# JiuTongBro/MultiView_Inpaint

Measured on AMD Instinct MI355X. Metric: Mpix/s fwd+bwd @1.5M Gauss 1080p, higher is better.
Workload: dtype f32; 1 GPU; rasterizer-with-depth fwd+bwd, one 1920x1080 view per GPU per step, N=1500000 Gaussians, sh_degree 3 (BASELINE.json configs[2] size, SURVEY.md §8d scene); gaussians=1500000, visible=1312313, num_rendered_D=14779663, tiles=8160, tile_list_max=2266, parallelism=views x1

## Files before the change

include/mvi_raster.h:

```cpp
#ifndef MVI_RASTER_H
#define MVI_RASTER_H

#include <stddef.h>
#include <stdint.h>

#ifdef __cplusplus
extern "C" {
#endif

#define MVI_OK 0
#define MVI_EINVAL (-1)
#define MVI_EHIP (-2)
#define MVI_ENOMEM (-3)

#define MVI_TILE 16

typedef struct mvi_raster_settings {
    int32_t image_height;
    int32_t image_width;
    float tanfovx;
    float tanfovy;
    float scale_modifier;
    int32_t sh_degree;
    int32_t prefiltered;
// ... 83 lines not shown
int mvi_raster_backward_geom_range(const mvi_raster_settings* s, int32_t P, int32_t M, int32_t first, int32_t count,
                                   const float* means3D, const float* shs, const float* colors_precomp, const float* scales,
                                   const float* rotations, const float* cov3D_precomp, const int32_t* radii, const void* geom,
                                   const float* grad_rows_scratch, float* dL_dmeans3D, float* dL_dmeans2D, float* dL_dopacity,
                                   float* dL_dshs, float* dL_dcolors, float* dL_dscales, float* dL_drotations, float* dL_dcov3D,
                                   void* stream);

typedef struct mvi_raster_views {
    const float* depths;
    const float* means2D;
    const float* cov3D_a;
    const float* cov3D_b;
    const float* conic_opacity;
    const float* rgbd;
    const uint32_t* tiles_touched;
    const uint8_t* clamped;
    const void* tile_ids_sorted;
    const uint32_t* point_list;
    const uint32_t* ranges;
    const float* final_T;
    const uint32_t* n_contrib;
    int32_t tile_id_bytes;
    const uint8_t* grad_support;
} mvi_raster_views;
int mvi_raster_get_views(int32_t P, int64_t num_rendered, int32_t image_width, int32_t image_height,
                         const void* geom, const void* binning, const void* image,
                         mvi_raster_views* out);
int mvi_raster_materialize_geom_views(const mvi_raster_settings* s, int32_t P, const float* means3D, const float* scales,
                                      const float* rotations, const float* cov3D_precomp, const int32_t* radii, void* geom,
                                      void* stream);
int mvi_raster_materialize_tile_ids(int32_t P, int64_t num_rendered, int32_t image_width, int32_t image_height,
                                    void* binning, const void* image, void* stream);

#define MVI_RASTER_NSTAGES 8
int mvi_raster_timing_enable(int enable);
int mvi_raster_timing_enable_stages(uint32_t stage_mask);
int mvi_raster_timing_read(float* ms_sum_host, int32_t* calls_host);
const char* mvi_raster_stage_name(int stage);

int mvi_raster_color_mode(int deferred);
int mvi_raster_forward_group(int group);
int mvi_raster_resolve_colors(const mvi_raster_settings* s, int32_t P, void* geom, size_t geom_bytes, void* stream);

int mvi_raster_binning_version(int version);
int mvi_raster_backward_mode(int dense);
int mvi_raster_dev_stamps(int pass, void* device_buffer);
int mvi_raster_dev_wave_sum9(const float* in, float* out, int n_waves, void* stream);

const char* mvi_raster_last_error(void);
const char* mvi_version(void);

#ifdef __cplusplus
}
#endif
#endif
```

multiview_inpaint_amd/_lib.py:

```python
import ctypes as C
import os
import re

_HERE = os.path.dirname(os.path.abspath(__file__))
LIB_PATH = os.environ.get("MVI_HIP_LIB") or os.path.join(_HERE, "csrc", "libmvi_hip.so")
LIB_OVERRIDDEN = bool(os.environ.get("MVI_HIP_LIB"))
if LIB_OVERRIDDEN:
    import sys as _sys
    _sys.stderr.write(f"[mvi] MVI_HIP_LIB is set: every kernel comes from {LIB_PATH}, not from the in-tree build\n")
INCLUDE_DIR = os.path.normpath(os.path.join(_HERE, "..", "include"))


class RasterSettings(C.Structure):
    _fields_ = [
        ("image_height", C.c_int32), ("image_width", C.c_int32),
        ("tanfovx", C.c_float), ("tanfovy", C.c_float), ("scale_modifier", C.c_float),
        ("sh_degree", C.c_int32), ("prefiltered", C.c_int32),
        ("bg", C.c_void_p), ("viewmatrix", C.c_void_p), ("projmatrix", C.c_void_p), ("campos", C.c_void_p),
    ]


class RasterViews(C.Structure):
    _fields_ = [(n, C.c_void_p) for n in (
        "depths", "means2D", "cov3D_a", "cov3D_b", "conic_opacity", "rgbd", "tiles_touched", "clamped",
        "tile_ids_sorted", "point_list", "ranges", "final_T", "n_contrib")] + [("tile_id_bytes", C.c_int32),
                                                                                   ("grad_support", C.c_void_p)]


class AdamGroup(C.Structure):
    _fields_ = [("param", C.c_void_p), ("grad", C.c_void_p), ("exp_avg", C.c_void_p), ("exp_avg_sq", C.c_void_p),
                ("n", C.c_int64), ("lr", C.c_float)]


class CompactTensor(C.Structure):
    _fields_ = [("in_", C.c_void_p), ("out", C.c_void_p), ("width", C.c_int32), ("packed_stride", C.c_int32)]


def declared_symbols():
    names = []
    for fn in sorted(os.listdir(INCLUDE_DIR)):
        if fn.endswith(".h"):
            src = open(os.path.join(INCLUDE_DIR, fn)).read()
            src = re.sub(r"/\*.*?\*/", "", src, flags=re.S)
            names += re.findall(r"\b(mvi_[a-z0-9_]+)\s*\(", src)
    return sorted(set(names))


def raster_source_digest():
    import hashlib
# ... 62 lines not shown
    L.mvi_raster_mark_visible.argtypes = [i32, vp, vp, vp, vp, vp]
    L.mvi_raster_get_views.restype = C.c_int
    L.mvi_raster_get_views.argtypes = [i32, i64, i32, i32, vp, vp, vp, C.POINTER(RasterViews)]
    L.mvi_raster_materialize_geom_views.restype = C.c_int
    L.mvi_raster_materialize_geom_views.argtypes = [C.POINTER(RasterSettings), i32] + [vp] * 7
    L.mvi_raster_materialize_tile_ids.restype = C.c_int
    L.mvi_raster_materialize_tile_ids.argtypes = [i32, i64, i32, i32, vp, vp, vp]
    L.mvi_raster_timing_enable.restype = C.c_int
    L.mvi_raster_timing_enable.argtypes = [C.c_int]
    L.mvi_raster_timing_enable_stages.restype = C.c_int
    L.mvi_raster_timing_enable_stages.argtypes = [C.c_uint32]
    L.mvi_raster_timing_read.restype = C.c_int
    L.mvi_raster_timing_read.argtypes = [C.POINTER(C.c_float), C.POINTER(C.c_int32)]
    L.mvi_raster_stage_name.restype = C.c_char_p
    L.mvi_raster_stage_name.argtypes = [C.c_int]
    L.mvi_raster_binning_version.restype = C.c_int
    L.mvi_raster_binning_version.argtypes = [C.c_int]
    L.mvi_raster_backward_mode.restype = C.c_int
    L.mvi_raster_backward_mode.argtypes = [C.c_int]
    L.mvi_raster_color_mode.restype = C.c_int
    L.mvi_raster_color_mode.argtypes = [C.c_int]
    L.mvi_raster_forward_group.restype = C.c_int
    L.mvi_raster_forward_group.argtypes = [C.c_int]
    L.mvi_raster_resolve_colors.restype = C.c_int
    L.mvi_raster_resolve_colors.argtypes = [C.POINTER(RasterSettings), i32, vp, sz, vp]
    L.mvi_raster_dev_stamps.restype = C.c_int
    L.mvi_raster_dev_stamps.argtypes = [C.c_int, vp]
    L.mvi_raster_dev_wave_sum9.restype = C.c_int
    L.mvi_raster_dev_wave_sum9.argtypes = [vp, vp, C.c_int, vp]
    _bind_unet_ops(L)
    _bind_train_ops(L)
    _bind_box_region(L)
    _lib = L
    return L


def _bind_unet_ops(L):
    try:
        from . import _unet_ops_bind
    except ImportError:
        return
    _unet_ops_bind.bind(L)


def _bind_train_ops(L):
    vp, i32, sz, f32 = C.c_void_p, C.c_int32, C.c_size_t, C.c_float
# ... 50 lines not shown
```

multiview_inpaint_amd/csrc/raster_api.hip:

```cpp
#include <cstdio>
#include <cstdlib>
#include <cstring>
#include <mutex>
#include <vector>

#include "raster_common.h"

static thread_local char g_err[512] = "";
static int g_dense_backward = [] { const char* e = getenv("MVI_RASTER_DENSE_BACKWARD"); return (e && e[0] == '1') ? 1 : 0; }();
static int g_defer_colors = [] { const char* e = getenv("MVI_RASTER_EAGER_COLORS"); return (e && e[0] == '1') ? 0 : 1; }();
namespace {
struct SegmentHint { const void* geom; int32_t P; int64_t segments; uint64_t stamp; };
constexpr int kSegmentHints = 64;
SegmentHint g_seg_hints[kSegmentHints] = {};
uint64_t g_seg_clock = 0;
std::mutex g_seg_mutex;
void remember_segments(const void* geom, int32_t P, int64_t segments) {
    std::lock_guard<std::mutex> lock(g_seg_mutex);
    int slot = 0;
    for (int i = 0; i < kSegmentHints; ++i) {
        if (g_seg_hints[i].geom == geom) { slot = i; break; }
        if (g_seg_hints[i].stamp < g_seg_hints[slot].stamp) slot = i;
    }
    g_seg_hints[slot] = {geom, P, segments, ++g_seg_clock};
// ... 81 lines not shown
    g_recs.clear();
    return MVI_OK;
}
const char* mvi_raster_stage_name(int i) {
    static const char* n[MVI_RASTER_NSTAGES] = {"preprocess_forward", "scan_block_sums", "duplicate_keys", "radix_sort",
                                                "tile_ranges", "render_forward", "render_backward", "preprocess_backward"};
    return (i >= 0 && i < MVI_RASTER_NSTAGES) ? n[i] : "";
}
int mvi_raster_dev_stamps(int pass, void* device_buffer) { mvi::set_dev_stamps(pass, device_buffer); return MVI_OK; }
int mvi_raster_dev_wave_sum9(const float* in, float* out, int n_waves, void* stream) {
    if (n_waves < 0 || (n_waves > 0 && (!in || !out))) return fail(MVI_EINVAL, "wave_sum9: NULL buffer or negative n_waves%s");
    if (mvi::launch_wave_sum9_probe(in, out, n_waves, (hipStream_t)stream)) return hip_fail("wave_sum9 probe", hipGetLastError());
    return MVI_OK;
}
int mvi_raster_backward_mode(int dense) {
    const int old = g_dense_backward;
    if (dense == 0 || dense == 1) g_dense_backward = dense;
    return old;
}
int mvi_raster_binning_version(int version) { return mvi::set_binning_version(version); }
int mvi_raster_forward_group(int group) {
    const int old = mvi::set_forward_group(group);
    return old < 0 ? fail(MVI_EINVAL, "forward group: no such instantiation of render_forward%s") : old;
}
int mvi_raster_color_mode(int deferred) {
    const int old = g_defer_colors;
    if (deferred == 0 || deferred == 1) g_defer_colors = deferred;
    return old;
}
int mvi_raster_resolve_colors(const mvi_raster_settings* s, int32_t P, void* geom, size_t geom_bytes, void* stream) {
    mvi::Frame f;
    if (int rc = make_frame(s, P, 0, f)) return rc;
    if (P == 0) return MVI_OK;
    if (!geom) return fail(MVI_EINVAL, "geom is NULL%s");
    mvi::GeomView g = mvi::carve_geom(geom, P);
    if (geom_bytes < g.bytes) return fail(MVI_ENOMEM, "geom scratch too small%s", "");
    if (mvi::launch_resolve_colors(f, g, (hipStream_t)stream)) return hip_fail("resolve_colors", hipGetLastError());
    return MVI_OK;
}
const char* mvi_version(void) { return "multiview_inpaint_amd 0.1.0 (gfx950)"; }

size_t mvi_raster_geom_bytes(int32_t P) { return mvi::carve_geom(nullptr, P).bytes; }
size_t mvi_raster_image_bytes(int32_t W, int32_t H) { return mvi::carve_image(nullptr, W, H).bytes; }
size_t mvi_raster_binning_bytes(int64_t D, int32_t W, int32_t H) { return mvi::carve_binning(nullptr, D, W, H).bytes; }

static int forward_geom_impl(const mvi_raster_settings* s, mvi::Frame& f, int32_t P, int32_t M, const float* means3D,
// ... 410 lines not shown
}

int mvi_raster_get_views(int32_t P, int64_t D, int32_t W, int32_t H, const void* geom, const void* binning,
                         const void* image, mvi_raster_views* out) {
    if (!out) return fail(MVI_EINVAL, "views is NULL%s");
    memset(out, 0, sizeof(*out));
    if (geom) {
        mvi::GeomView g = mvi::carve_geom(const_cast<void*>(geom), P);
        out->depths = g.depths; out->means2D = reinterpret_cast<const float*>(g.xy);
        out->cov3D_a = reinterpret_cast<const float*>(g.cov_a); out->cov3D_b = reinterpret_cast<const float*>(g.cov_b);
        out->conic_opacity = reinterpret_cast<const float*>(g.conic_opacity); out->rgbd = reinterpret_cast<const float*>(g.rgbd);
        out->tiles_touched = g.tiles_touched; out->clamped = g.clamped;
        out->grad_support = g.touched;
    }
    if (binning) {
        mvi::BinningView b = mvi::carve_binning(const_cast<void*>(binning), D, W, H);
        int fin = b.passes & 1;
        out->tile_ids_sorted = b.keys[fin]; out->point_list = b.vals[fin];
        out->tile_id_bytes = b.key_bytes;
    }
    if (image) {
        mvi::ImageView im = mvi::carve_image(const_cast<void*>(image), W, H);
        out->ranges = im.ranges; out->final_T = im.final_T; out->n_contrib = im.n_contrib;
    }
    return MVI_OK;
}

int mvi_raster_materialize_geom_views(const mvi_raster_settings* s, int32_t P, const float* means3D, const float* scales,
                                      const float* rotations, const float* cov3D_precomp, const int32_t* radii, void* geom,
                                      void* stream) {
    mvi::Frame f;
    if (int rc = make_frame(s, P, 0, f)) return rc;
    if (P == 0) return MVI_OK;
    if (!means3D || !radii || !geom) return fail(MVI_EINVAL, "NULL means3D/radii/geom in materialize_geom_views%s");
    if (((scales == nullptr) || (rotations == nullptr)) == (cov3D_precomp == nullptr))
        return fail(MVI_EINVAL, "Please provide exactly one of either scale/rotation pair or precomputed 3D covariance!%s");
    mvi::GeomView g = mvi::carve_geom(geom, P);
    if (mvi::launch_materialize_geom_views(f, means3D, scales, rotations, cov3D_precomp, radii, g, (hipStream_t)stream))
        return hip_fail("materialize_geom_views", hipGetLastError());
    return MVI_OK;
}

int mvi_raster_materialize_tile_ids(int32_t P, int64_t D, int32_t W, int32_t H, void* binning, const void* image, void* stream) {
    if (P < 0 || D < 0 || W < 0 || H < 0) return fail(MVI_EINVAL, "negative size in materialize_tile_ids%s");
    if (P == 0 || D == 0) return MVI_OK;
    if (!binning || !image) return fail(MVI_EINVAL, "NULL scratch in materialize_tile_ids%s");
// ... 9 lines not shown
```

multiview_inpaint_amd/csrc/raster_binning.hip:

```cpp
#include "raster_common.h"
#include "raster_scan.h"

namespace mvi {

__global__ __launch_bounds__(256) void zero_fill_kernel(uint4* __restrict__ p, size_t n16) {
    for (size_t i = (size_t)blockIdx.x * 256 + threadIdx.x; i < n16; i += (size_t)gridDim.x * 256) p[i] = make_uint4(0u, 0u, 0u, 0u);
}
int launch_zero_fill(void* p, size_t bytes, hipStream_t st) {
    if (bytes == 0) return 0;
    const size_t n16 = (bytes + 15) / 16;
    size_t blocks = (n16 + 255) / 256;
    if (blocks > 256 * 32) blocks = 256 * 32;
    hipLaunchKernelGGL(zero_fill_kernel, dim3((unsigned)blocks), dim3(256), 0, st, (uint4*)p, n16);
    return hipGetLastError() == hipSuccess ? 0 : MVI_EHIP;
}

__global__ __launch_bounds__(1024) void scan_block_sums_kernel(const uint32_t* __restrict__ sums,
                                                               uint32_t* __restrict__ offsets, int n) {
    __shared__ uint32_t s_wave[16];
    __shared__ uint32_t s_carry;
    const int tid = threadIdx.x;
    const uint32_t total = row_excl_scan_1024(sums, offsets, n, tid, s_wave, &s_carry);
    if (tid == 0) offsets[n] = total;
}
// ... 325 lines not shown
    {
        StageTimer tm(kStDup, st);
        hipLaunchKernelGGL((emit_pairs_kernel<KeyT>), dim3(nblk), dim3(kBlock), 0, st, f, g, g.dvals[0], g.perm_offsets,
                           keys[0], b.vals[0]);
    }
    int cur = 0;
    {
        StageTimer tm(kStSort, st);
        int shift = 0;
        for (int p = 0; p < b.passes; ++p) {
            const int left = b.passes - p;
            const int bits = (b.key_bits - shift + left - 1) / left;
            cur = radix_pass<kSortWavesD, KeyT>(keys, b.vals, cur, D, shift, bits, b.block_hist, b.digit_tot, b.nsort, st);
            shift += bits;
        }
    }
    int nrb = (int)((D + kBlock - 1) / kBlock);
    StageTimer tm(kStRanges, st);
    hipLaunchKernelGGL((tile_ranges_kernel<KeyT>), dim3(nrb), dim3(kBlock), 0, st, keys[cur], D, im.ranges);
    return hipGetLastError() == hipSuccess ? 0 : MVI_EHIP;
}

int launch_binning(const Frame& f, GeomView g, BinningView b, ImageView im, int64_t D, hipStream_t st) {
    size_t tiles = (size_t)f.gx * f.gy;
    if (launch_zero_fill(im.ranges, 8 * tiles, st)) return MVI_EHIP;
    if (D <= 0 || f.P <= 0) return 0;
    return b.key_bytes == 2 ? binning_typed<uint16_t>(f, g, b, im, D, st) : binning_typed<uint32_t>(f, g, b, im, D, st);
}

}
```

multiview_inpaint_amd/csrc/raster_binning2.hip:

```cpp
#include <cstdlib>

#include "raster_common.h"
#include "raster_scan.h"

namespace mvi {

static int g_binning_version = [] { const char* e = getenv("MVI_BINNING_LEGACY"); return (e && e[0] == '1') ? 1 : 2; }();
bool binning_v2_enabled() { return g_binning_version == 2; }
int set_binning_version(int v) {
    const int old = g_binning_version;
    if (v == 1 || v == 2) g_binning_version = v;
    return old;
}

__device__ __forceinline__ uint32_t block_excl_scan256(uint32_t v, int tid, uint32_t* s_w4, uint32_t* total) {
    const int lane = tid & 63, wave = tid >> 6;
    const uint32_t inc = wave_incl_scan(v, lane);
    if (wave < 4 && lane == 63) s_w4[wave] = inc;
    __syncthreads();
    uint32_t off = 0;
#pragma unroll
    for (int w = 0; w < 3; ++w) if (w < wave) off += s_w4[w];
    if (total) *total = s_w4[0] + s_w4[1] + s_w4[2] + s_w4[3];
    __syncthreads();
// ... 314 lines not shown
    if (!load_chunk(chunk_first, col_start, gx, tid, s_first, s_col, ck)) return;
    const uint32_t last = ck.seg1 ? ck.seg1 - 1u : 0u;
    uint32_t yhs[kEx2Items];
#pragma unroll
    for (int k = 0; k < kEx2Items; ++k) yhs[k] = seg_yh[min(ck.seg0 + (uint32_t)(k * kExThreads + tid), last)];
#pragma unroll
    for (int k = 0; k < kEx2Items; ++k) {
        const uint32_t i = ck.seg0 + (uint32_t)(k * kExThreads + tid);
        if (i < ck.seg1) {
            const uint32_t yh = yhs[k];
            const uint32_t y0 = yh & 255u, h = (yh >> 8) + 1u;
            atomicAdd(&s_d[y0], 1u);
            atomicSub(&s_d[y0 + h], 1u);
        }
    }
    __syncthreads();
    const uint32_t v = tid < 256 ? s_d[tid] : 0u;
    const uint32_t ex = block_excl_scan256(v, tid, s_w4, nullptr);
    if (tid < gy) row_table[(size_t)tid * stride + blockIdx.x] = ex + v;
}

__global__ __launch_bounds__(1024) void row_scan_kernel(int gx, const uint32_t* __restrict__ chunk_first,
                                                        uint32_t* __restrict__ row_table, int stride,
                                                        uint32_t* __restrict__ row_tot, uint32_t* __restrict__ col_rel) {
    __shared__ uint32_t s_first[257];
    __shared__ uint32_t s_wave[16];
    __shared__ uint32_t s_carry;
    const int tid = threadIdx.x;
    if (tid <= gx) s_first[tid] = chunk_first[tid];
    const int n = (int)chunk_first[gx];
    uint32_t* row = row_table + (size_t)blockIdx.x * stride;
    const uint32_t total = row_excl_scan_1024(row, row, n, tid, s_wave, &s_carry);
    __syncthreads();
    uint32_t* cr = col_rel + (size_t)blockIdx.x * (gx + 1);
    if (tid < gx) cr[tid] = __hip_atomic_load(row + s_first[tid], __ATOMIC_RELAXED, __HIP_MEMORY_SCOPE_AGENT);
    if (tid == 0) { cr[gx] = total; row_tot[blockIdx.x] = total; }
}

struct ExpandArgs {
    int n_items;
    int nbins;
    int gx;
    const uint32_t* order;
    const uint2* rect_sorted;
    const uint32_t* chunk_first;
    const uint32_t* col_start;
    const uint32_t* seg_idx_in;
    const uint16_t* seg_yh_in;
    const uint32_t* col_rel;
    uint32_t* ranges;
    const uint32_t* table;
// ... 188 lines not shown

int launch_binning2_level1(const Frame& f, GeomView g, hipStream_t st) {
    if (f.P <= 0) return 0;
    {
        StageTimer tm(kStSort, st);
#define MVI_DS_PASS(PASS, SRC, DST)                                                                                              \
        hipLaunchKernelGGL(depth_count_kernel, dim3(g.nds), dim3(kDsThreads), 0, st, g.dkeys[SRC], f.P, 8 * PASS, g.ds_table,     \
                           g.ds_super[PASS & 1]);                                                                                 \
        hipLaunchKernelGGL((depth_scatter_kernel<PASS>), dim3(g.nds), dim3(kDsThreads), 0, st, g.dkeys[SRC], g.dvals[SRC],        \
                           g.dkeys[DST], g.dvals[DST], f.P, g.ds_table, g.ds_super[PASS & 1], g.nsuper,                           \
                           PASS < 3 ? g.ds_super[(PASS + 1) & 1] : (uint32_t*)nullptr, g.rect, g.rect_sorted);
        MVI_DS_PASS(0, 0, 1) MVI_DS_PASS(1, 1, 0) MVI_DS_PASS(2, 0, 1) MVI_DS_PASS(3, 1, 0)
#undef MVI_DS_PASS
    }
    StageTimer tm(kStDup, st);
    hipLaunchKernelGGL(column_count_kernel, dim3(g.nblk1), dim3(kExThreads), 0, st, f.P, f.gx, g.rect_sorted, g.col_table,
                       g.nblk1);
    hipLaunchKernelGGL(columns_scan_kernel, dim3(f.gx), dim3(1024), 0, st, g.col_table, g.nblk1, g.nblk1, g.col_tot, f.gx,
                       g.arrivals, g.chunk_first, g.col_start);
    return hipGetLastError() == hipSuccess ? 0 : MVI_EHIP;
}

int launch_binning2(const Frame& f, GeomView g, BinningView b, ImageView im, int64_t D, int64_t segments, hipStream_t st) {
    const size_t tiles = (size_t)f.gx * f.gy;
    if (D <= 0 || f.P <= 0) return launch_zero_fill(im.ranges, 8 * tiles, st);
    const bool wide = f.gx > 128 || f.gy > 128;
    ExpandArgs a1{};
    a1.n_items = f.P; a1.nbins = f.gx; a1.gx = f.gx;
    a1.order = g.dvals[0]; a1.rect_sorted = g.rect_sorted;
    a1.table = g.col_table; a1.tot = g.col_tot; a1.stride = g.nblk1;
    a1.out_idx = b.vals[0]; a1.out_aux = (uint16_t*)b.keys[0];
    a1.stamps = g_dev_stamps[0];
    {
        StageTimer tm(kStDup, st);
        if (wide)
            hipLaunchKernelGGL((expand_scatter_kernel<1, 256, kExItems, 64 * 256>), dim3(g.nblk1), dim3(kExThreads), 0, st, a1);
        else hipLaunchKernelGGL((expand_scatter_kernel<1, 128, kExItems, 64 * 128>), dim3(g.nblk1), dim3(kExThreads), 0, st, a1);
    }
    int nchunk = b.nsort;
    if (segments > 0 && segments <= D) nchunk = (int)min((int64_t)b.nsort, segments / kEx2Chunk + f.gx + 1);
    ExpandArgs a2{};
    a2.nbins = f.gy; a2.gx = f.gx;
    a2.chunk_first = g.chunk_first; a2.col_start = g.col_start;
    a2.seg_idx_in = b.vals[0]; a2.seg_yh_in = (const uint16_t*)b.keys[0];
    a2.col_rel = b.col_rel; a2.ranges = im.ranges;
    a2.table = b.block_hist; a2.tot = b.digit_tot; a2.stride = b.nsort;
    a2.out_idx = b.vals[1];
    a2.stamps = g_dev_stamps[1];
    StageTimer tm(kStSort, st);
    hipLaunchKernelGGL(row_count_kernel, dim3(nchunk), dim3(kExThreads), 0, st, f.gx, f.gy, g.chunk_first, g.col_start,
                       (const uint16_t*)b.keys[0], b.block_hist, b.nsort);
    hipLaunchKernelGGL(row_scan_kernel, dim3(f.gy), dim3(1024), 0, st, f.gx, g.chunk_first, b.block_hist, b.nsort,
                       b.digit_tot, b.col_rel);
    if (f.gy <= kEx2SmallNB)
        hipLaunchKernelGGL((expand_scatter_kernel<2, kEx2SmallNB, kEx2Items, kEx2SmallCap>), dim3(nchunk), dim3(kExThreads), 0,
                           st, a2);
    else if (f.gy <= 128)
        hipLaunchKernelGGL((expand_scatter_kernel<2, 128, kEx2Items, 64 * 128>), dim3(nchunk), dim3(kExThreads), 0, st, a2);
    else hipLaunchKernelGGL((expand_scatter_kernel<2, 256, kEx2Items, 64 * 256>), dim3(nchunk), dim3(kExThreads), 0, st, a2);
    return hipGetLastError() == hipSuccess ? 0 : MVI_EHIP;
}

}
```

multiview_inpaint_amd/csrc/raster_common.h:

```cpp
#pragma once
#include <hip/hip_runtime.h>
#include <stdint.h>
#include <stddef.h>
#include <type_traits>

#include "../../include/mvi_raster.h"

namespace mvi {

constexpr int kTile = MVI_TILE;
constexpr int kBlock = 256;
constexpr int kPB = 64;
constexpr float kNearZ = 0.2f;
constexpr float kLowpass = 0.3f;
constexpr float kFrustumClamp = 1.3f;
constexpr float kLambdaFloor = 0.1f;
constexpr float kAlphaMax = 0.99f;
constexpr float kAlphaMin = 1.0f / 255.0f;
constexpr float kTEps = 0.0001f;
constexpr float kDepthSentinel = 15.0f;

constexpr int kSortItems = 8;
constexpr int kSortWavesP = 4;
constexpr int kSortWavesD = 8;
// ... 12 lines not shown
    const float* campos;
    const float* bg;
    const float* shs_rest = nullptr;
    int raw = 0;
    int bin_v2 = 0;
    int defer_colors = 0;
};

constexpr int kDsThreads = 256;
constexpr int kDsItems = 8;
constexpr int kDsTile = kDsThreads * kDsItems;
constexpr int kDsSuper = 16;
constexpr int kExThreads = 512;
constexpr int kExItems = 4;
constexpr int kExChunk = kExThreads * kExItems;
constexpr int kEx2Items = 3;
constexpr int kEx2Chunk = kExThreads * kEx2Items;
constexpr int kEx2SmallNB = 80;
constexpr int kEx2SmallCap = 7168;
bool binning_v2_enabled();
void set_dev_stamps(int pass, void* buf);
int set_binning_version(int v);
int set_forward_group(int g);
inline bool binning_v2_ok(int gx, int gy) { return gx <= 256 && gy <= 256 && binning_v2_enabled(); }

struct ColorSource {
    const float* means3D;
    const float* shs;
    const float* shs_rest;
    int32_t M, deg, raw;
    int32_t deferred;
    int32_t vec16;
};

struct GeomView {
    float* depths;
    float2* xy;
    float4* cov_a;
    float2* cov_b;
    float4* conic_opacity;
    float4* rgbd;
    uint32_t* tiles_touched;
    uint2* rect;
    uint8_t* clamped;
    uint8_t* front;
    struct ColorSource* color_src;
    uint8_t* touched;
    uint32_t* block_sums;
    uint32_t* block_offsets;
    uint32_t* dkeys[2];
    uint32_t* dvals[2];
    uint32_t* dhist;
    uint32_t* dtot;
    uint32_t* perm_sums;
    uint32_t* perm_offsets;
    uint2* rect_sorted;
    uint32_t* col_table;
    uint32_t* col_tot;
    uint32_t* seg_sums;
    uint32_t* chunk_first;
    uint32_t* col_start;
    uint32_t* arrivals;
    uint32_t* ds_table;
    uint32_t* ds_super[2];
    int nds, nsuper;
    int nblk1;
    int nsortP;
    size_t bytes;
};
struct ImageView {
    uint32_t* ranges;
    float* final_T;
    uint32_t* n_contrib;
    size_t bytes;
};
struct BinningView {
    void* keys[2];
    int key_bytes;
    uint32_t* vals[2];
    uint32_t* block_hist;
    uint32_t* digit_tot;
    int nsort;
    int passes;
    int key_bits;
    int v2;
    uint32_t* col_rel;
    size_t bytes;
};

inline size_t align256(size_t x) { return (x + 255) & ~size_t(255); }

inline GeomView carve_geom(void* base, int P) {
    GeomView g;
    char* p = (char*)base;
// ... 27 lines not shown
    g.nblk1 = (int)((n + kExChunk - 1) / kExChunk);
    g.col_table = (uint32_t*)take(4 * 256 * (size_t)g.nblk1);
    g.col_tot = (uint32_t*)take(4 * 256);
    g.seg_sums = (uint32_t*)take(4 * npre);
    g.chunk_first = (uint32_t*)take(4 * 257);
    g.col_start = (uint32_t*)take(4 * 257);
    g.arrivals = (uint32_t*)take(4);
    g.nds = (int)((n + kDsTile - 1) / kDsTile);
    g.nsuper = (g.nds + kDsSuper - 1) / kDsSuper;
    g.ds_table = (uint32_t*)take(4 * 256 * (size_t)g.nds);
    g.ds_super[0] = (uint32_t*)take(4 * 256 * (size_t)g.nsuper);
    g.ds_super[1] = (uint32_t*)take(4 * 256 * (size_t)g.nsuper);
    g.bytes = o;
    return g;
}
inline ImageView carve_image(void* base, int W, int H) {
    ImageView v;
    char* p = (char*)base;
    size_t o = 0;
    size_t tiles = (size_t)((W + kTile - 1) / kTile) * ((H + kTile - 1) / kTile);
    size_t px = (size_t)W * H;
    auto take = [&](size_t b) { char* r = p ? p + o : nullptr; o += align256(b); return r; };
    v.ranges = (uint32_t*)take(8 * (tiles ? tiles : 1));
    v.final_T = (float*)take(4 * (px ? px : 1));
    v.n_contrib = (uint32_t*)take(4 * (px ? px : 1));
    v.bytes = o;
    return v;
}
inline int tile_bits(int W, int H) {
    unsigned tiles = (unsigned)(((W + kTile - 1) / kTile) * ((H + kTile - 1) / kTile));
    int b = 0;
    while ((1u << b) < tiles && b < 31) ++b;
    return b > 0 ? b : 1;
}
inline BinningView carve_binning(void* base, int64_t D, int W, int H) {
    BinningView v;
    char* p = (char*)base;
    size_t o = 0;
    size_t n = (size_t)(D > 0 ? D : 1);
    v.nsort = sort_blocks(n, kSortWavesD);
    v.key_bits = tile_bits(W, H);
    v.passes = (v.key_bits + 7) / 8;
    auto take = [&](size_t b) { char* r = p ? p + o : nullptr; o += align256(b); return r; };
    const unsigned tiles = (unsigned)(((W + kTile - 1) / kTile) * ((H + kTile - 1) / kTile));
    v.key_bytes = tiles <= 65536u ? 2 : 4;
    const int gx = (W + kTile - 1) / kTile, gy = (H + kTile - 1) / kTile;
    v.v2 = binning_v2_ok(gx, gy) ? 1 : 0;
    v.col_rel = nullptr;
    if (v.v2) {
        v.nsort = (int)((n / kEx2Chunk + (size_t)gx + 1 + 3) / 4 * 4);
// ... 196 lines not shown
}
__device__ __forceinline__ bool color_pending(float4 cd) { return cd.x < 0.0f || cd.y < 0.0f || cd.z < 0.0f; }

template <int CTRL, int ROW_MASK>
__device__ __forceinline__ float dpp_add(float v) {
    int t = __builtin_amdgcn_update_dpp(0, __float_as_int(v), CTRL, ROW_MASK, 0xf, true);
    return v + __int_as_float(t);
}
__device__ __forceinline__ float wave_sum_to_lane63(float v) {
    v = dpp_add<0xb1, 0xf>(v);
    v = dpp_add<0x4e, 0xf>(v);
    v = dpp_add<0x114, 0xf>(v);
    v = dpp_add<0x118, 0xf>(v);
    v = dpp_add<0x142, 0xa>(v);
    v = dpp_add<0x143, 0xc>(v);
    return v;
}
__device__ __forceinline__ float row_sum_to_lane15(float v) {
    v = dpp_add<0xb1, 0xf>(v);
    v = dpp_add<0x4e, 0xf>(v);
    v = dpp_add<0x114, 0xf>(v);
    v = dpp_add<0x118, 0xf>(v);
    return v;
}
__device__ __forceinline__ uint32_t wave_sum_u32(uint32_t v) {
    for (int o = 32; o > 0; o >>= 1) v += __shfl_xor(v, o);
    return v;
}

enum Stage { kStPreFwd = 0, kStScan, kStDup, kStSort, kStRanges, kStRenderFwd, kStRenderBwd, kStPreBwd };
void stage_begin(int stage, hipStream_t st);
void stage_end(int stage, hipStream_t st);
struct StageTimer {
    int stage; hipStream_t st;
    StageTimer(int s, hipStream_t q) : stage(s), st(q) { stage_begin(stage, st); }
    ~StageTimer() { stage_end(stage, st); }
};

constexpr int kMaxZero = 10;
struct ZeroRegions {
    float* head[kMaxZero];
    uint4* body[kMaxZero];
    float* tail[kMaxZero];
    uint32_t n_head[kMaxZero], n_body[kMaxZero], n_tail[kMaxZero];
    int n = 0;
    bool overflow = false;
// ... 74 lines not shown
```

multiview_inpaint_amd/csrc/raster_render.hip:

```cpp
#include <cstdlib>

#include "raster_common.h"
#include "raster_render_shared.h"

namespace mvi {


template <int G, bool AUX>
__global__ __launch_bounds__(kBlock) __attribute__((amdgpu_waves_per_eu(G == 1 ? 1 : 6, G == 1 ? 8 : 6))) void render_forward_kernel(
    Frame f, const uint32_t* __restrict__ ranges, const uint32_t* __restrict__ point_list,
    const float2* __restrict__ xy, float4* rgbd, const float4* __restrict__ conic_opacity,
    float* __restrict__ final_T, uint32_t* __restrict__ n_contrib, float* __restrict__ out_color,
    float* __restrict__ out_depth, ZeroRegions zero, const ColorSource* __restrict__ color_src, uint8_t* clamped,
    float* __restrict__ out_expected_depth, float* __restrict__ out_alpha) {
    __shared__ float2 s_xy[kBlock];
    __shared__ float s_t2[kBlock];
    __shared__ float4 s_co[kBlock];
    __shared__ float4 s_cd[kBlock];
    __shared__ float4 w_s[4][3][64];
    const int tid = threadIdx.x, wave = tid >> 6, lane = tid & 63;
    zero_share(zero, tid, kBlock);
    const int tile = xcd_band_tile(blockIdx.x, f.gx * f.gy);
    const int tile_y = tile / f.gx, tile_x = tile - tile_y * f.gx;
    const int qx0 = tile_x * kTile + 8 * (wave & 1), qy0 = tile_y * kTile + 8 * (wave >> 1);
    const int pxi = qx0 + (lane & 7), pyi = qy0 + (lane >> 3);
    const bool inside = pxi < f.W && pyi < f.H;
    const float pfx = (float)pxi, pfy = (float)pyi;
    const uint32_t r0 = ranges[2 * tile], r1 = ranges[2 * tile + 1];
    int todo = (int)(r1 - r0);
    const int rounds = (todo + kBlock - 1) / kBlock;

    float T = inside ? 1.0f : 0.0f;
    float T_out = 1.0f, C2 = 0.f, Dp = kDepthSentinel, Tc = 1.0f;
    [[maybe_unused]] float Dexp = 0.f;
    f2 C01 = {0.f, 0.f};
    uint32_t last = 0;

// ... 66 lines not shown
            } else {
                const float4* g = &w_s[wave][0][0];
                int k = 0;
                float chain = 0.0f;
                if (cnt >= G) {
                    do {
                        float4 a = g[0], co = g[64], cd = g[128];
#pragma unroll
                        for (int j = 0; j < G; ++j) {
                            const int jn = j + 1 < G ? j + 1 : j;
                            const float4 an = g[jn], con = g[64 + jn], cdn = g[128 + jn];
                            __builtin_amdgcn_sched_barrier(0);
                            chain = entry(a, co, cd, chain);
                            a = an; co = con; cd = cdn;
                        }
                        k += G; g += G;
                    } while ((k + G <= cnt) & (ballot64(T > 0.0f) != 0ull));
                }
                if (k < cnt && ballot64(T > 0.0f) != 0ull)
                    for (; k < cnt; ++k, ++g) chain = entry(g[0], g[64], g[128], chain);
            }
        }
    }
    if (inside) {
        size_t pix = (size_t)pyi * f.W + pxi, hw = (size_t)f.H * f.W;
        final_T[pix] = T_out;
        n_contrib[pix] = last;
        out_color[pix] = C01.x + T_out * f.bg[0];
        out_color[hw + pix] = C01.y + T_out * f.bg[1];
        out_color[2 * hw + pix] = C2 + T_out * f.bg[2];
        out_depth[pix] = Tc < 0.5f ? Dp : kDepthSentinel;
        if constexpr (AUX) {
            out_expected_depth[pix] = Dexp;
            out_alpha[pix] = 1.0f - T_out;
        }
    }
}

constexpr int kFrontTiles = 4;
constexpr int kFrontMax = 1024;
__global__ __launch_bounds__(kBlock) void mark_front_kernel(int tiles, const uint32_t* __restrict__ ranges,
                                                            const uint32_t* __restrict__ point_list, uint8_t* __restrict__ front,
                                                            int n_front, const ColorSource* __restrict__ color_src, int gx,
                                                            int every) {
    if (!color_src->deferred) return;
    const int tid = threadIdx.x;
    const int sx = (gx + every - 1) / every;
#pragma unroll
    for (int t = 0; t < kFrontTiles; ++t) {
        const int j = blockIdx.x * kFrontTiles + t;
        const int tile = every == 1 ? j : (j / sx) * every * gx + (j % sx) * every;
        if (tile >= tiles) break;
        const uint32_t r0 = ranges[2 * tile], r1 = ranges[2 * tile + 1];
        const uint32_t n = min(r1 - r0, (uint32_t)n_front);
        for (uint32_t e = tid; e < n; e += kBlock) front[point_list[r0 + e]] = 1;
    }
}
constexpr int kMarkedPer = 4;
// ... 13 lines not shown
            if (((w >> (8 * k)) & 0xFFu) && i0 + k < f.P) s_id[atomicAdd(&s_n, 1u)] = (uint32_t)(i0 + k);
    }
    __syncthreads();
    const uint32_t total = s_n;
    for (uint32_t i = tid; i < total; i += kBlock) {
        const uint32_t id = s_id[i];
        const float4 cd = g.rgbd[id];
        if (color_pending(cd)) resolve_color(cs, f.campos, id, cd.w, g.rgbd, g.clamped);
    }
}

constexpr int kForwardGroupDefault = 4;
static bool forward_group_built(int g) { return g == 1 || g == 4; }
static int g_forward_group = [] { const char* e = getenv("MVI_RASTER_FORWARD_GROUP"); const int v = e ? atoi(e) : 0;
                                  return forward_group_built(v) ? v : kForwardGroupDefault; }();
int set_forward_group(int g) {
    const int old = g_forward_group;
    if (g == -1) return old;
    if (g != 0 && !forward_group_built(g)) return MVI_EINVAL;
    g_forward_group = g == 0 ? kForwardGroupDefault : g;
    return old;
}

int launch_zero_fill(void* p, size_t bytes, hipStream_t st);
int launch_render_forward(const Frame& f, GeomView g, BinningView b, ImageView im, int64_t D,
                          float* out_color, float* out_depth, hipStream_t st, float* zero_rows, float* out_expected_depth,
                          float* out_alpha) {
    if ((out_expected_depth == nullptr) != (out_alpha == nullptr)) return MVI_EINVAL;
    ZeroRegions z;
    if (zero_rows) {
        z.add(zero_rows, (size_t)f.P * kGradRow);
        z.add(g.touched, ((size_t)f.P + 15) / 16 * 4);
    }
    if (f.W <= 0 || f.H <= 0) return launch_zero_regions(z, st);
    const uint32_t* plist = b.vals[b.passes & 1];
    const unsigned blocks = (unsigned)(f.gx * f.gy);
    if (f.defer_colors && D > 0) {
        static const int n_front = [] { const char* e = getenv("MVI_RASTER_FRONT_ENTRIES"); const int v = e ? atoi(e) : kBlock;
                                        return v < 0 ? 0 : (v > kFrontMax ? kFrontMax : v); }();
        static const int every = [] { const char* e = getenv("MVI_RASTER_FRONT_EVERY"); const int v = e ? atoi(e) : 2; return v < 1 ? 1 : v; }();
        if (n_front > 0) {
            const unsigned sampled = (unsigned)(((f.gx + every - 1) / every) * ((f.gy + every - 1) / every));
            hipLaunchKernelGGL(mark_front_kernel, dim3((sampled + kFrontTiles - 1) / kFrontTiles), dim3(kBlock), 0, st, (int)blocks,
                               im.ranges, plist, g.front, n_front, g.color_src, f.gx, every);
            hipLaunchKernelGGL(resolve_marked_kernel, dim3((f.P + kBlock * kMarkedPer - 1) / (kBlock * kMarkedPer)), dim3(kBlock), 0, st,
                               f, g);
        }
    }
#define MVI_RENDER_FORWARD(G, AUX)                                                                                          \
    hipLaunchKernelGGL((render_forward_kernel<G, AUX>), dim3(blocks), dim3(kBlock), 0, st, f, im.ranges, plist, g.xy, g.rgbd, \
                       g.conic_opacity, im.final_T, im.n_contrib, out_color, out_depth, z, g.color_src, g.clamped,            \
                       out_expected_depth, out_alpha)
    switch (g_forward_group * 2 + (out_alpha ? 1 : 0)) {
        case 2: MVI_RENDER_FORWARD(1, false); break;
        case 3: MVI_RENDER_FORWARD(1, true); break;
        case 8: MVI_RENDER_FORWARD(4, false); break;
        case 9: MVI_RENDER_FORWARD(4, true); break;
        default: return MVI_EINVAL;
    }
#undef MVI_RENDER_FORWARD
    return hipGetLastError() == hipSuccess ? 0 : MVI_EHIP;
}

__global__ __launch_bounds__(256) void zero_regions_kernel(ZeroRegions z) { zero_share(z, threadIdx.x, 256); }
int launch_zero_regions(const ZeroRegions& z, hipStream_t st) {
    if (z.n == 0) return 0;
    hipLaunchKernelGGL(zero_regions_kernel, dim3(2048), dim3(256), 0, st, z);
    return hipGetLastError() == hipSuccess ? 0 : MVI_EHIP;
}


__global__ __launch_bounds__(64) void wave_sum9_probe_kernel(const float* __restrict__ in, float* __restrict__ out) {
    const int lane = threadIdx.x;
    const float* x = in + (size_t)blockIdx.x * 9 * 64 + lane;
    const float s = wave_sum9(x[0], x[64], x[128], x[192], x[256], x[320], x[384], x[448], x[512]);
    if (wave_sum9_owner(lane)) out[blockIdx.x * 9 + wave_sum9_moment(lane)] = s;
}
int launch_wave_sum9_probe(const float* in, float* out, int n_waves, hipStream_t st) {
    if (n_waves <= 0) return 0;
    hipLaunchKernelGGL(wave_sum9_probe_kernel, dim3(n_waves), dim3(64), 0, st, in, out);
    return hipGetLastError() == hipSuccess ? 0 : MVI_EHIP;
}

#ifndef MVI_RB_WAVES
#define MVI_RB_WAVES 5
#endif
__global__ __launch_bounds__(kB2) __attribute__((amdgpu_waves_per_eu(MVI_RB_WAVES, MVI_RB_WAVES))) void render_backward_kernel(
    Frame f, const uint32_t* __restrict__ ranges, const uint32_t* __restrict__ point_list,
    const float2* __restrict__ xy, const float4* __restrict__ rgbd, const float4* __restrict__ conic_opacity,
    const float* __restrict__ final_T, const uint32_t* __restrict__ n_contrib,
    const float* __restrict__ dL_dpix, float* __restrict__ grad_rows, uint8_t* __restrict__ touched, ZeroRegions zero) {
#pragma clang fp contract(off)
    zero_share(zero, threadIdx.x, kB2);
    __shared__ float4 s_ent[3][kB2];
    __shared__ float s_acc[kB2][9];
    __shared__ uint32_t s_blast[2];
    const int tid = threadIdx.x, wave = tid >> 6, lane = tid & 63;
    const int tile = xcd_band_tile(blockIdx.x, f.gx * f.gy);
    const int tile_y = tile / f.gx, tile_x = tile - tile_y * f.gx;
    const int hx0 = tile_x * kTile, hy0 = tile_y * kTile + 8 * wave;
    const int pxi = hx0 + (lane & 15), py0 = hy0 + 2 * (lane >> 4), py1 = py0 + 1;
    const bool in0 = pxi < f.W && py0 < f.H, in1 = pxi < f.W && py1 < f.H;
    const float pfx = (float)pxi;
    const f2 pfy = {(float)py0, (float)py1};
    const uint32_t r0 = ranges[2 * tile];
    const size_t hw = (size_t)f.H * f.W, pix0 = (size_t)py0 * f.W + pxi, pix1 = pix0 + f.W;

    const f2 T_final = {in0 ? final_T[pix0] : 0.0f, in1 ? final_T[pix1] : 0.0f};
    f2 T = T_final;
    const uint32_t last0 = in0 ? n_contrib[pix0] : 0u, last1 = in1 ? n_contrib[pix1] : 0u;
    f2 A_dot = {0.f, 0.f};
    f2 dp0 = {0.f, 0.f}, dp1 = {0.f, 0.f}, dp2 = {0.f, 0.f};
    if (in0) { dp0.x = dL_dpix[pix0]; dp1.x = dL_dpix[hw + pix0]; dp2.x = dL_dpix[2 * hw + pix0]; }
    if (in1) { dp0.y = dL_dpix[pix1]; dp1.y = dL_dpix[hw + pix1]; dp2.y = dL_dpix[2 * hw + pix1]; }
    const f2 bg_dot = f.bg[0] * dp0 + f.bg[1] * dp1 + f.bg[2] * dp2;
    const f2 bg_term = -T_final * bg_dot;
    uint32_t wave_last = max(last0, last1);
    for (int o = 32; o > 0; o >>= 1) wave_last = max(wave_last, (uint32_t)__shfl_xor((int)wave_last, o));
    if (lane == 0) s_blast[wave] = wave_last;
    __syncthreads();
    const int total = (int)max(s_blast[0], s_blast[1]);
// ... 95 lines not shown
                }
            }
            asm volatile("s_waitcnt lgkmcnt(0)" ::: "memory");
            __builtin_amdgcn_wave_barrier();
            const int comp = lane & 15;
#pragma unroll 4
            for (int it = 0; it < 16; ++it) {
                const int e = wave * 64 + it * 4 + (lane >> 4);
                const uint32_t id = e < n ? __float_as_uint(s_ent[0][e].w) : 0xFFFFFFFFu;
                if (id == 0xFFFFFFFFu || comp >= 9) continue;
                atomicAdd(&grad_rows[(size_t)id * kRow + comp], s_acc[e][comp]);
                if (comp == 0) touched[id] = 1;
            }
        }
    }
}

int launch_render_backward(const Frame& f, GeomView g, BinningView b, ImageView im, int64_t D,
                           const float* dL_dpix, float* grad_rows, hipStream_t st, const ZeroRegions* zero) {
    ZeroRegions z;
    if (zero) z = *zero;
    if (f.W <= 0 || f.H <= 0 || D <= 0) return launch_zero_regions(z, st);
    const uint32_t* plist = b.vals[b.passes & 1];
    hipLaunchKernelGGL(render_backward_kernel, dim3(f.gx * f.gy), dim3(kB2), 0, st, f, im.ranges, plist, g.xy,
                       g.rgbd, g.conic_opacity, im.final_T, im.n_contrib, dL_dpix, grad_rows, g.touched, z);
    return hipGetLastError() == hipSuccess ? 0 : MVI_EHIP;
}

}
```

Baseline: 2498 Mpix/s.

## Schedule backward render tiles heaviest-first via per-band tile-class queues

The forward kernel now takes the maximum contributor count of each tile and buckets the tile into one of 16 cost classes per XCD band, appending its id to a per-class queue through an atomic. The backward kernel maps block ids through these queues so the most expensive tiles launch first within each band, which is meant to reduce the tail imbalance at the end of the backward pass. In exchange it adds a wave max reduction, a syncthreads and an atomic to the forward pass, a slightly larger zero fill, and an extra lookup per backward block. The new order is on by default, with an env/API switch back to plain band order.

Result: faster. 2586 Mpix/s, median of 6 (+3.5%).

```diff
diff --git a/include/mvi_raster.h b/include/mvi_raster.h
--- a/include/mvi_raster.h
+++ b/include/mvi_raster.h
@@ -129,6 +129,8 @@
     const uint32_t* n_contrib;
     int32_t tile_id_bytes;
     const uint8_t* grad_support;
+    const uint32_t* tile_class_count;
+    const uint32_t* tile_class_queue;
 } mvi_raster_views;
 int mvi_raster_get_views(int32_t P, int64_t num_rendered, int32_t image_width, int32_t image_height,
                          const void* geom, const void* binning, const void* image,
@@ -147,6 +149,7 @@
 
 int mvi_raster_color_mode(int deferred);
 int mvi_raster_forward_group(int group);
+int mvi_raster_backward_order(int order);
 int mvi_raster_resolve_colors(const mvi_raster_settings* s, int32_t P, void* geom, size_t geom_bytes, void* stream);
 
 int mvi_raster_binning_version(int version);
diff --git a/multiview_inpaint_amd/_lib.py b/multiview_inpaint_amd/_lib.py
--- a/multiview_inpaint_amd/_lib.py
+++ b/multiview_inpaint_amd/_lib.py
@@ -24,7 +24,9 @@
     _fields_ = [(n, C.c_void_p) for n in (
         "depths", "means2D", "cov3D_a", "cov3D_b", "conic_opacity", "rgbd", "tiles_touched", "clamped",
         "tile_ids_sorted", "point_list", "ranges", "final_T", "n_contrib")] + [("tile_id_bytes", C.c_int32),
-                                                                                   ("grad_support", C.c_void_p)]
+                                                                                   ("grad_support", C.c_void_p),
+                                                                                   ("tile_class_count", C.c_void_p),
+                                                                                   ("tile_class_queue", C.c_void_p)]
 
 
 class AdamGroup(C.Structure):
@@ -133,6 +135,8 @@
     L.mvi_raster_color_mode.argtypes = [C.c_int]
     L.mvi_raster_forward_group.restype = C.c_int
     L.mvi_raster_forward_group.argtypes = [C.c_int]
+    L.mvi_raster_backward_order.restype = C.c_int
+    L.mvi_raster_backward_order.argtypes = [C.c_int]
     L.mvi_raster_resolve_colors.restype = C.c_int
     L.mvi_raster_resolve_colors.argtypes = [C.POINTER(RasterSettings), i32, vp, sz, vp]
     L.mvi_raster_dev_stamps.restype = C.c_int
diff --git a/multiview_inpaint_amd/csrc/raster_api.hip b/multiview_inpaint_amd/csrc/raster_api.hip
--- a/multiview_inpaint_amd/csrc/raster_api.hip
+++ b/multiview_inpaint_amd/csrc/raster_api.hip
@@ -127,6 +127,10 @@
 int mvi_raster_forward_group(int group) {
     const int old = mvi::set_forward_group(group);
     return old < 0 ? fail(MVI_EINVAL, "forward group: no such instantiation of render_forward%s") : old;
+}
+int mvi_raster_backward_order(int order) {
+    const int old = mvi::set_backward_order(order);
+    return old < 0 ? fail(MVI_EINVAL, "backward order: 1 (heaviest first), 0 (plain band order) or -1 (query)%s") : old;
 }
 int mvi_raster_color_mode(int deferred) {
     const int old = g_defer_colors;
@@ -583,6 +587,7 @@
     if (image) {
         mvi::ImageView im = mvi::carve_image(const_cast<void*>(image), W, H);
         out->ranges = im.ranges; out->final_T = im.final_T; out->n_contrib = im.n_contrib;
+        out->tile_class_count = im.class_count; out->tile_class_queue = im.class_queue;
     }
     return MVI_OK;
 }
diff --git a/multiview_inpaint_amd/csrc/raster_binning.hip b/multiview_inpaint_amd/csrc/raster_binning.hip
--- a/multiview_inpaint_amd/csrc/raster_binning.hip
+++ b/multiview_inpaint_amd/csrc/raster_binning.hip
@@ -371,8 +371,7 @@
 }
 
 int launch_binning(const Frame& f, GeomView g, BinningView b, ImageView im, int64_t D, hipStream_t st) {
-    size_t tiles = (size_t)f.gx * f.gy;
-    if (launch_zero_fill(im.ranges, 8 * tiles, st)) return MVI_EHIP;
+    if (launch_zero_fill(im.ranges, ranges_and_counts_bytes(im), st)) return MVI_EHIP;
     if (D <= 0 || f.P <= 0) return 0;
     return b.key_bytes == 2 ? binning_typed<uint16_t>(f, g, b, im, D, st) : binning_typed<uint32_t>(f, g, b, im, D, st);
 }
diff --git a/multiview_inpaint_amd/csrc/raster_binning2.hip b/multiview_inpaint_amd/csrc/raster_binning2.hip
--- a/multiview_inpaint_amd/csrc/raster_binning2.hip
+++ b/multiview_inpaint_amd/csrc/raster_binning2.hip
@@ -360,11 +360,13 @@
 
 __global__ __launch_bounds__(1024) void row_scan_kernel(int gx, const uint32_t* __restrict__ chunk_first,
                                                         uint32_t* __restrict__ row_table, int stride,
-                                                        uint32_t* __restrict__ row_tot, uint32_t* __restrict__ col_rel) {
+                                                        uint32_t* __restrict__ row_tot, uint32_t* __restrict__ col_rel,
+                                                        uint32_t* __restrict__ class_count) {
     __shared__ uint32_t s_first[257];
     __shared__ uint32_t s_wave[16];
     __shared__ uint32_t s_carry;
     const int tid = threadIdx.x;
+    if (blockIdx.x == 0 && tid < kTileBands * kTileClasses) class_count[tid] = 0u;
     if (tid <= gx) s_first[tid] = chunk_first[tid];
     const int n = (int)chunk_first[gx];
     uint32_t* row = row_table + (size_t)blockIdx.x * stride;
@@ -599,8 +601,7 @@
 }
 
 int launch_binning2(const Frame& f, GeomView g, BinningView b, ImageView im, int64_t D, int64_t segments, hipStream_t st) {
-    const size_t tiles = (size_t)f.gx * f.gy;
-    if (D <= 0 || f.P <= 0) return launch_zero_fill(im.ranges, 8 * tiles, st);
+    if (D <= 0 || f.P <= 0) return launch_zero_fill(im.ranges, ranges_and_counts_bytes(im), st);
     const bool wide = f.gx > 128 || f.gy > 128;
     ExpandArgs a1{};
     a1.n_items = f.P; a1.nbins = f.gx; a1.gx = f.gx;
@@ -628,7 +629,7 @@
     hipLaunchKernelGGL(row_count_kernel, dim3(nchunk), dim3(kExThreads), 0, st, f.gx, f.gy, g.chunk_first, g.col_start,
                        (const uint16_t*)b.keys[0], b.block_hist, b.nsort);
     hipLaunchKernelGGL(row_scan_kernel, dim3(f.gy), dim3(1024), 0, st, f.gx, g.chunk_first, b.block_hist, b.nsort,
-                       b.digit_tot, b.col_rel);
+                       b.digit_tot, b.col_rel, im.class_count);
     if (f.gy <= kEx2SmallNB)
         hipLaunchKernelGGL((expand_scatter_kernel<2, kEx2SmallNB, kEx2Items, kEx2SmallCap>), dim3(nchunk), dim3(kExThreads), 0,
                            st, a2);
diff --git a/multiview_inpaint_amd/csrc/raster_common.h b/multiview_inpaint_amd/csrc/raster_common.h
--- a/multiview_inpaint_amd/csrc/raster_common.h
+++ b/multiview_inpaint_amd/csrc/raster_common.h
@@ -58,6 +58,7 @@
 void set_dev_stamps(int pass, void* buf);
 int set_binning_version(int v);
 int set_forward_group(int g);
+int set_backward_order(int order);
 inline bool binning_v2_ok(int gx, int gy) { return gx <= 256 && gy <= 256 && binning_v2_enabled(); }
 
 struct ColorSource {
@@ -104,8 +105,15 @@
     int nsortP;
     size_t bytes;
 };
+constexpr int kTileBands = 8;
+constexpr int kTileClasses = 16;
+constexpr int kTileClassWidth = 32;
+__host__ __device__ inline int tile_queue_stride(int tiles) { return (tiles + kTileBands - 1) / kTileBands + 1; }
+template <typename T> __host__ __device__ inline T* tile_class_queues(T* class_count) { return class_count + kTileBands * kTileClasses; }
 struct ImageView {
     uint32_t* ranges;
+    uint32_t* class_count;
+    uint32_t* class_queue;
     float* final_T;
     uint32_t* n_contrib;
     size_t bytes;
@@ -179,10 +187,15 @@
     size_t px = (size_t)W * H;
     auto take = [&](size_t b) { char* r = p ? p + o : nullptr; o += align256(b); return r; };
     v.ranges = (uint32_t*)take(8 * (tiles ? tiles : 1));
+    v.class_count = (uint32_t*)take(4 * kTileBands * kTileClasses);
+    v.class_queue = (uint32_t*)take(4 * (size_t)kTileBands * kTileClasses * (size_t)tile_queue_stride((int)tiles));
     v.final_T = (float*)take(4 * (px ? px : 1));
     v.n_contrib = (uint32_t*)take(4 * (px ? px : 1));
     v.bytes = o;
     return v;
+}
+inline size_t ranges_and_counts_bytes(const ImageView& v) {
+    return (size_t)((char*)v.class_count - (char*)v.ranges) + 4 * (size_t)kTileBands * kTileClasses;
 }
 inline int tile_bits(int W, int H) {
     unsigned tiles = (unsigned)(((W + kTile - 1) / kTile) * ((H + kTile - 1) / kTile));
@@ -425,6 +438,19 @@
     v = dpp_add<0x114, 0xf>(v);
     v = dpp_add<0x118, 0xf>(v);
     return v;
+}
+template <int CTRL>
+__device__ __forceinline__ uint32_t dpp_umax(uint32_t v) {
+    return max(v, (uint32_t)__builtin_amdgcn_update_dpp(0, (int)v, CTRL, 0xf, 0xf, true));
+}
+__device__ __forceinline__ uint32_t wave_umax(uint32_t v) {
+    v = dpp_umax<0xb1>(v);
+    v = dpp_umax<0x4e>(v);
+    v = dpp_umax<0x114>(v);
+    v = dpp_umax<0x118>(v);
+    const uint32_t a = (uint32_t)__builtin_amdgcn_readlane((int)v, 15), b = (uint32_t)__builtin_amdgcn_readlane((int)v, 31);
+    const uint32_t c = (uint32_t)__builtin_amdgcn_readlane((int)v, 47), d = (uint32_t)__builtin_amdgcn_readlane((int)v, 63);
+    return max(max(a, b), max(c, d));
 }
 __device__ __forceinline__ uint32_t wave_sum_u32(uint32_t v) {
     for (int o = 32; o > 0; o >>= 1) v += __shfl_xor(v, o);
diff --git a/multiview_inpaint_amd/csrc/raster_render.hip b/multiview_inpaint_amd/csrc/raster_render.hip
--- a/multiview_inpaint_amd/csrc/raster_render.hip
+++ b/multiview_inpaint_amd/csrc/raster_render.hip
@@ -1,4 +1,5 @@
 #include <cstdlib>
+#include <mutex>
 
 #include "raster_common.h"
 #include "raster_render_shared.h"
@@ -12,7 +13,8 @@
     const float2* __restrict__ xy, float4* rgbd, const float4* __restrict__ conic_opacity,
     float* __restrict__ final_T, uint32_t* __restrict__ n_contrib, float* __restrict__ out_color,
     float* __restrict__ out_depth, ZeroRegions zero, const ColorSource* __restrict__ color_src, uint8_t* clamped,
-    float* __restrict__ out_expected_depth, float* __restrict__ out_alpha) {
+    float* __restrict__ out_expected_depth, float* __restrict__ out_alpha, uint32_t* __restrict__ class_count) {
+    __shared__ uint32_t s_wmax[4];
     __shared__ float2 s_xy[kBlock];
     __shared__ float s_t2[kBlock];
     __shared__ float4 s_co[kBlock];
@@ -125,6 +127,15 @@
             }
         }
     }
+    const uint32_t wmax = wave_umax(last);
+    if (lane == 0) s_wmax[wave] = wmax;
+    __syncthreads();
+    uint32_t cls = 0, slot = 0;
+    if (tid == 0) {
+        const uint32_t m = max(max(s_wmax[0], s_wmax[1]), max(s_wmax[2], s_wmax[3]));
+        cls = (blockIdx.x & (kTileBands - 1)) * kTileClasses + min((uint32_t)(kTileClasses - 1), m / kTileClassWidth);
+        slot = atomicAdd(&class_count[cls], 1u);
+    }
     if (inside) {
         size_t pix = (size_t)pyi * f.W + pxi, hw = (size_t)f.H * f.W;
         final_T[pix] = T_out;
@@ -137,6 +148,10 @@
             out_expected_depth[pix] = Dexp;
             out_alpha[pix] = 1.0f - T_out;
         }
+    }
+    if (tid == 0) {
+        const uint32_t stride = (uint32_t)tile_queue_stride(f.gx * f.gy);
+        if (slot < stride) tile_class_queues(class_count)[(size_t)cls * stride + slot] = (uint32_t)tile;
     }
 }
 
@@ -196,6 +211,39 @@
     return old;
 }
 
+constexpr int kBackwardOrderDefault = 1;
+static int g_backward_order = [] { const char* e = getenv("MVI_RASTER_BACKWARD_ORDER");
+                                   return e && (e[0] == '0' || e[0] == '1') && e[1] == 0 ? e[0] - '0' : kBackwardOrderDefault; }();
+int set_backward_order(int order) {
+    const int old = g_backward_order;
+    if (order == -1) return old;
+    if (order != 0 && order != 1) return MVI_EINVAL;
+    g_backward_order = order;
+    return old;
+}
+namespace {
+struct QueueNote { const void* image; int W, H; uint64_t stamp; };
+constexpr int kQueueNotes = 64;
+QueueNote g_queue_notes[kQueueNotes] = {};
+uint64_t g_queue_clock = 0;
+std::mutex g_queue_mutex;
+void note_queue_filled(const void* image, int W, int H) {
+    std::lock_guard<std::mutex> lock(g_queue_mutex);
+    int slot = 0;
+    for (int i = 0; i < kQueueNotes; ++i) {
+        if (g_queue_notes[i].image == image) { slot = i; break; }
+        if (g_queue_notes[i].stamp < g_queue_notes[slot].stamp) slot = i;
+    }
+    g_queue_notes[slot] = {image, W, H, ++g_queue_clock};
+}
+bool queue_filled(const void* image, int W, int H) {
+    std::lock_guard<std::mutex> lock(g_queue_mutex);
+    for (int i = 0; i < kQueueNotes; ++i)
+        if (g_queue_notes[i].image == image && g_queue_notes[i].stamp) return g_queue_notes[i].W == W && g_queue_notes[i].H == H;
+    return false;
+}
+}
+
 int launch_zero_fill(void* p, size_t bytes, hipStream_t st);
 int launch_render_forward(const Frame& f, GeomView g, BinningView b, ImageView im, int64_t D,
                           float* out_color, float* out_depth, hipStream_t st, float* zero_rows, float* out_expected_depth,
@@ -224,7 +272,7 @@
 #define MVI_RENDER_FORWARD(G, AUX)                                                                                          \
     hipLaunchKernelGGL((render_forward_kernel<G, AUX>), dim3(blocks), dim3(kBlock), 0, st, f, im.ranges, plist, g.xy, g.rgbd, \
                        g.conic_opacity, im.final_T, im.n_contrib, out_color, out_depth, z, g.color_src, g.clamped,            \
-                       out_expected_depth, out_alpha)
+                       out_expected_depth, out_alpha, im.class_count)
     switch (g_forward_group * 2 + (out_alpha ? 1 : 0)) {
         case 2: MVI_RENDER_FORWARD(1, false); break;
         case 3: MVI_RENDER_FORWARD(1, true); break;
@@ -233,7 +281,9 @@
         default: return MVI_EINVAL;
     }
 #undef MVI_RENDER_FORWARD
-    return hipGetLastError() == hipSuccess ? 0 : MVI_EHIP;
+    if (hipGetLastError() != hipSuccess) return MVI_EHIP;
+    note_queue_filled(im.ranges, f.W, f.H);
+    return 0;
 }
 
 __global__ __launch_bounds__(256) void zero_regions_kernel(ZeroRegions z) { zero_share(z, threadIdx.x, 256); }
@@ -259,18 +309,36 @@
 #ifndef MVI_RB_WAVES
 #define MVI_RB_WAVES 5
 #endif
+__device__ __forceinline__ int heaviest_first_tile(int bid, int tiles, const uint32_t* __restrict__ class_count) {
+    const int queue_stride = tile_queue_stride(tiles);
+    const int x = bid & (kTileBands - 1);
+    uint32_t rel = (uint32_t)bid >> 3;
+    const uint32_t* cc = class_count + x * kTileClasses;
+    int c = kTileClasses - 1;
+#pragma unroll
+    for (int k = kTileClasses - 1; k > 0; --k) {
+        const uint32_t n = cc[k];
+        if (c == k && rel >= n) { rel -= n; c = k - 1; }
+    }
+    rel = min(rel, (uint32_t)(queue_stride - 1));
+    const uint32_t t = tile_class_queues(class_count)[(size_t)(x * kTileClasses + c) * queue_stride + rel];
+    return (int)min(t, (uint32_t)(tiles - 1));
+}
+template <bool QUEUE>
 __global__ __launch_bounds__(kB2) __attribute__((amdgpu_waves_per_eu(MVI_RB_WAVES, MVI_RB_WAVES))) void render_backward_kernel(
     Frame f, const uint32_t* __restrict__ ranges, const uint32_t* __restrict__ point_list,
     const float2* __restrict__ xy, const float4* __restrict__ rgbd, const float4* __restrict__ conic_opacity,
     const float* __restrict__ final_T, const uint32_t* __restrict__ n_contrib,
-    const float* __restrict__ dL_dpix, float* __restrict__ grad_rows, uint8_t* __restrict__ touched, ZeroRegions zero) {
+    const float* __restrict__ dL_dpix, float* __restrict__ grad_rows, uint8_t* __restrict__ touched, ZeroRegions zero,
+    const uint32_t* __restrict__ class_count) {
 #pragma clang fp contract(off)
     zero_share(zero, threadIdx.x, kB2);
     __shared__ float4 s_ent[3][kB2];
     __shared__ float s_acc[kB2][9];
     __shared__ uint32_t s_blast[2];
     const int tid = threadIdx.x, wave = tid >> 6, lane = tid & 63;
-    const int tile = xcd_band_tile(blockIdx.x, f.gx * f.gy);
+    const int tile = QUEUE ? heaviest_first_tile(blockIdx.x, f.gx * f.gy, class_count)
+                           : xcd_band_tile(blockIdx.x, f.gx * f.gy);
     const int tile_y = tile / f.gx, tile_x = tile - tile_y * f.gx;
     const int hx0 = tile_x * kTile, hy0 = tile_y * kTile + 8 * wave;
     const int pxi = hx0 + (lane & 15), py0 = hy0 + 2 * (lane >> 4), py1 = py0 + 1;
@@ -412,8 +480,12 @@
     if (zero) z = *zero;
     if (f.W <= 0 || f.H <= 0 || D <= 0) return launch_zero_regions(z, st);
     const uint32_t* plist = b.vals[b.passes & 1];
-    hipLaunchKernelGGL(render_backward_kernel, dim3(f.gx * f.gy), dim3(kB2), 0, st, f, im.ranges, plist, g.xy,
-                       g.rgbd, g.conic_opacity, im.final_T, im.n_contrib, dL_dpix, grad_rows, g.touched, z);
+    if (g_backward_order == 1 && queue_filled(im.ranges, f.W, f.H))
+        hipLaunchKernelGGL(render_backward_kernel<true>, dim3(f.gx * f.gy), dim3(kB2), 0, st, f, im.ranges, plist, g.xy, g.rgbd,
+                           g.conic_opacity, im.final_T, im.n_contrib, dL_dpix, grad_rows, g.touched, z, im.class_count);
+    else
+        hipLaunchKernelGGL(render_backward_kernel<false>, dim3(f.gx * f.gy), dim3(kB2), 0, st, f, im.ranges, plist, g.xy, g.rgbd,
+                           g.conic_opacity, im.final_T, im.n_contrib, dL_dpix, grad_rows, g.touched, z, (const uint32_t*)nullptr);
     return hipGetLastError() == hipSuccess ? 0 : MVI_EHIP;
 }
 
```
